# Matrixeigs/PowerSystemsReliabilityAssessment

Hardware: AMD Instinct MI355X
Metric: Monte Carlo DC-OPF scenarios/sec (RTS-24 HL2 non-sequential) (higher is better)
Workload: dtype f64

## Files before the change

powersystemsreliabilityassessment_amd/csrc/relmc_kernels.hip:

```cpp
#include "relmc_devfn.h"
#include "relmc_shape_rts24.h"

namespace relmc {


constexpr int kPrioBit = 12;
constexpr int kMinWaves = 2;
#define DINF __builtin_inf()
#define RELOAD_FENCE() __asm__ volatile("" ::: "memory")
#define SLOT_FENCE() __builtin_amdgcn_sched_barrier(0)
#ifdef RELMC_PASS_NOUNROLL
#define PASS_LOOP _Pragma("nounroll")
#else
#define PASS_LOOP
#endif
constexpr int kPfMask = 0xc0;
constexpr int kPfMaskWide = 0xc6;
#define PFSITE(k) (((PF_MASK >> (k)) & 1) != 0)
constexpr int kShadowMask = 0xff;
constexpr int kShadowMaskWide = 0xff;
constexpr int kNormSplitMask = 0xff;
constexpr int kNormSplitMaskWide = 0;
#ifdef RELMC_ZERO_EXPLICIT
constexpr bool kZeroBySlot = false;
#else
constexpr bool kZeroBySlot = true;
#endif
#ifdef RELMC_FILL_LOOP
constexpr bool kFillBySlot = false;
#else
constexpr bool kFillBySlot = true;
#endif
#define PASS_IDLE(d) (((d).x & 0xffffu) == ((d).y >> 16))
#define PASS_IDLE_INV(d) ((d).y != 0u)
#ifdef RELMC_PHASE_TIMING
#define PT_DECL unsigned long long pt_[8] = {0, 0, 0, 0, 0, 0, 0, 0}, ptn_[2] = {0, 0}; unsigned long long pt0_ = __builtin_readcyclecounter();
#define PT_MARK(k) { const unsigned long long n_ = __builtin_readcyclecounter(); pt_[k] += n_ - pt0_; pt0_ = n_; }
#define PT_TRIP(k) ptn_[k] += 1;
#define PT_FLUSH if (a.timing && lane == 0) { for (int k = 0; k < 8; ++k) a.timing[((size_t)blockIdx.x * WPB + (tid >> 6)) * 8 + k] = pt_[k]; \
                                              for (int k = 0; k < 2; ++k) a.timing[(size_t)gridDim.x * WPB * 8 + ((size_t)blockIdx.x * WPB + (tid >> 6)) * 2 + k] = ptn_[k]; }
#else
#define PT_DECL
#define PT_MARK(k)
#define PT_TRIP(k)
#define PT_FLUSH
#endif
#if defined(RELMC_PHASE_TIMING) && defined(RELMC_PT_INIT)
#undef PT_MARK
#define PT_MARK(k) { const unsigned long long n_ = __builtin_readcyclecounter(); pt_[(k) == 7 ? 7 : 6] += n_ - pt0_; pt0_ = n_; }
#define PT_IMARK(k) { const unsigned long long n_ = __builtin_readcyclecounter(); pt_[k] += n_ - pt0_; pt0_ = n_; }
#else
#define PT_IMARK(k)
#endif

template <int MODE_, class TL, class SH = ShapeDynamic>
__global__ void __launch_bounds__(64 * TL::WPB, kMinWaves) relmc_eval_kernel(const DevCaseT<TL>* __restrict__ gcase, const EvalArgs a)
{
    constexpr int MODE = MODE_ == 5 ? 0 : (MODE_ == 6 ? 4 : MODE_);
    constexpr bool DENSE = MODE_ == 6;
    constexpr int PAIR_MASK = TL::RW == 16 ? kRpairMask : kRpairMaskWide;
#define PAIRSITE(k) (((PAIR_MASK >> (k)) & 1) != 0)
    constexpr int PF_MASK = TL::RW == 16 ? kPfMask : kPfMaskWide;
    constexpr bool SHADOW = (((TL::RW == 16 ? kShadowMask : kShadowMaskWide) >> MODE) & 1) != 0;
    constexpr bool NSPLIT = (((TL::RW == 16 ? kNormSplitMask : kNormSplitMaskWide) >> MODE) & 1) != 0;
    constexpr bool LSHARE = (((TL::RW == 16 ? kLineRcpShareMask : kLineRcpShareMaskWide) >> MODE) & 1) != 0 && PAIRSITE(0) && PAIRSITE(2) && PAIRSITE(6);
    constexpr bool ZSLOT = kZeroBySlot && (SH::kMask & SH::grp_nl) != 0 && (SH::kMask & SH::grp_ninj) != 0;
    constexpr bool FSLOT = kFillBySlot && !DENSE && (SH::kMask & SH::grp_nzero_res) != 0 && (SH::kMask & SH::grp_nfill_bus) != 0;
    constexpr bool FBUS = FSLOT && SH::nfill_bus > 0;
    constexpr int RW = TL::RW, BS = TL::BS, LS = TL::LS, IS = TL::IS, NBT = TL::NBT, WPB = TL::WPB, SPW = TL::SPW, OW = TL::OW;
    using DevCase = DevCaseT<TL>;
    using Partial = PartialT<TL>;
    extern __shared__ __attribute__((aligned(16))) unsigned char smem[];
    constexpr uint32_t OPT_BYTES = 128;
    double* const OPT = reinterpret_cast<double*>(smem);
#define A_(k, name) OPT[k]
    DevCase& C = *reinterpret_cast<DevCase*>(smem + OPT_BYTES);
    const DevCase& TASKSRC = *gcase;
    const DevCase& TABL = C;
    const DevCase& TABI = (RW == 64) ? *gcase : C;
    const DevCase& TABG = (RW == 64) ? *gcase : C;
    const int tid = threadIdx.x, lane = tid & 63, rlane = lane & (RW - 1), row = tid / RW;
    const uint32_t case_bytes = a.case_bytes;
    {
        const uint32_t* src = reinterpret_cast<const uint32_t*>(gcase);
        uint32_t* dst = reinterpret_cast<uint32_t*>(smem + OPT_BYTES);
        if (tid == 0) { OPT[0] = a.feastol; OPT[1] = a.gradtol; OPT[2] = a.comptol; OPT[3] = a.costtol; OPT[4] = a.xi; OPT[5] = a.sigma;
                        OPT[6] = a.z0; OPT[7] = a.alpha_min; OPT[8] = a.max_stepsize; OPT[9] = a.fail_threshold; }
        if constexpr (FSLOT) {
            constexpr uint32_t LB0 = offsetof(DevCase, l_blk) / 4, LBN = sizeof(DevCase::l_blk) / 4, LF0 = offsetof(DevCase, l_blk_fill) / 4;
            static_assert(offsetof(DevCase, l_blk) % 4 == 0 && sizeof(DevCase::l_blk) % 4 == 0 && offsetof(DevCase, l_blk_fill) % 4 == 0, "l_blk and l_blk_fill are copied as 32-bit words");
            for (uint32_t i = tid; i < case_bytes / 4; i += 64 * WPB) dst[i] = src[i - LB0 < LBN ? LF0 + (i - LB0) : i];
        } else
        for (uint32_t i = tid; i < case_bytes / 4; i += 64 * WPB) dst[i] = src[i];
    }
    __syncthreads();
    double* const W = reinterpret_cast<double*>(smem + OPT_BYTES + ((case_bytes + 15u) & ~15u)) + (size_t)row * SHAPE(scen_doubles, a.scen_doubles);
    const int nlp = SHAPE(nl, C.nl), nip = SHAPE(ninj, C.ninj);
    double* const LR = W;
    double* const IR = W + 4 * (nlp + 1);
    const int maxdeg0 = SHAPE(maxdeg0, C.maxdeg_s[0]), maxdeg1 = SHAPE(maxdeg1, C.maxdeg_s[1]), maxinj0 = SHAPE(maxinj0, C.maxinj_s[0]), maxinj1 = SHAPE(maxinj1, C.maxinj_s[1]);
    double* const Stash = W + SHAPE(stash_off, a.stash_off) + 2 * rlane;
    const double* const StashJ = W + SHAPE(stash_off, a.stash_off);
    double* const Lam = W + SHAPE(stash_off, a.stash_off) + 2 * IS * RW + 2;
    uint32_t* const OB = reinterpret_cast<uint32_t*>(Lam + NBT);

    const int ng = SHAPE(ng, C.ng), ncomp = C.ncomp, nb = SHAPE(nb, C.nb);
    const bool bwd_all_half = SHAPE(bwd_all_half, __builtin_amdgcn_readfirstlane((uint32_t)(C.bwd_half != 0 ? 1u : 0u)) != 0);
    const int off_rhs = SHAPE(off_rhs, C.off_rhs), npu = SHAPE(npass_upd, C.npass_upd), npi = SHAPE(npass_inv, C.npass_inv), npass = SHAPE(npass, C.npass), nzero = SHAPE(nzero, C.nzero), npuh = SHAPE(npass_upd, C.npass_upd) - SHAPE(npass_updq, C.npass_updq), npuf = npuh - SHAPE(npass_updh, C.npass_updh);
    const double base = C.base_mva;
    const double eps = 2.220446049250313e-16;

    uint32_t linfo[LS]; int lpart[LS];
#pragma unroll
    for (int s = 0; s < LS; ++s) { const int l = RW * s + rlane; linfo[s] = C.l_info[l]; lpart[s] = C.l_partner[l]; }
    constexpr bool LTAB_LDS = (MODE == 1 || MODE == 2 || MODE == 4);
    constexpr bool ITAB_REG = RW == 64;
    double lbv_[LS], lrv_[LS], ihi_[IS], ilo_[IS];
#pragma unroll
    for (int s = 0; s < LS; ++s) { lbv_[s] = LTAB_LDS ? 0.0 : TABL.l_b[RW * s + rlane]; lrv_[s] = LTAB_LDS ? 0.0 : TABL.l_rate[RW * s + rlane]; }
#pragma unroll
    for (int s = 0; s < IS; ++s) { ihi_[s] = ITAB_REG ? TABI.i_tab[RW * s + rlane][0] : 0.0; ilo_[s] = ITAB_REG ? TABI.i_tab[RW * s + rlane][1] : 0.0; }
#define lb(s) (LTAB_LDS ? TABL.l_b[RW * (s) + rlane] : lbv_[s])
#define lr(s) (LTAB_LDS ? TABL.l_rate[RW * (s) + rlane] : lrv_[s])
#define IHL(s, j) (ITAB_REG ? d2{ihi_[s], ilo_[s]} : ld2(TABI.i_tab[j]))
#define ICOST(s, j) TABI.i_tab[j][2]
#define PLIST(t, bi) TABG.b_line8[bi]
#define JLIST(t, bi) TABG.b_inj8[bi]
    uint32_t iinfo[IS];
#pragma unroll
    for (int s = 0; s < IS; ++s) iinfo[s] = C.i_info[RW * s + rlane];
    int vb[BS];
#pragma unroll
    for (int t = 0; t < BS; ++t) vb[t] = FBUS ? (int)gcase->b_lane_fill[RW * t + rlane] : (int)C.b_lane[RW * t + rlane];

    Partial& PA = reinterpret_cast<Partial*>(a.partial)[(size_t)blockIdx.x * (64 * WPB) + tid];
    {
        PA.dns = 0.0; PA.dns2 = 0.0;
#pragma unroll
        for (int s = 0; s < IS; ++s) { PA.shed[s] = 0.0; PA.cf_inj[s] = 0; }
#pragma unroll
        for (int s = 0; s < LS; ++s) PA.cf_line[s] = 0;
        PA.n = 0; PA.nfail = 0; PA.nsing = 0; PA.ninf = 0; PA.nnc = 0; PA.iters = 0; PA.pad = 0;
    }
    uint32_t acc_n = 0, acc_it = 0;

    PT_DECL
    const int64_t ngroups = (a.n + SPW - 1) / SPW;
    const int64_t gwave = (int64_t)blockIdx.x * WPB + (tid >> 6);
    const int64_t gstride = (int64_t)gridDim.x * WPB;
    const bool prio_first = a.prio_mode == 1 ? blockIdx.x < (gridDim.x >> 1) : (a.prio_mode == 2 ? ((tid >> 8) & 1) == 0 : false);
    if (a.prio_mode != 0 && !prio_first) __builtin_amdgcn_s_setprio(1);
    constexpr bool WINDOWED = (MODE == 0 && RW == 16);
    uint32_t* const WIN = reinterpret_cast<uint32_t*>(smem + OPT_BYTES + ((case_bytes + 15u) & ~15u)) +
                          (size_t)SPW * WPB * SHAPE(scen_doubles, a.scen_doubles) * 2 + (size_t)(tid >> 6) * 256;
    uint8_t* const WINL = reinterpret_cast<uint8_t*>(smem + OPT_BYTES + ((case_bytes + 15u) & ~15u)) +
                          ((size_t)SPW * WPB * SHAPE(scen_doubles, a.scen_doubles) * 2 + (size_t)WPB * 256) * 4 + (size_t)(tid >> 6) * 64;
    int64_t wb_begin = gwave, wb_end = ngroups, wb_step = gstride;
    if (WINDOWED) {
        wb_begin = ngroups * gwave / gstride; wb_end = ngroups * (gwave + 1) / gstride; wb_step = 16;
    }
    static_assert(!WINDOWED || 80 + 4 * WPB <= OPT_BYTES, "one word per wavefront behind the ten option doubles");
    int* const TP = reinterpret_cast<int*>(smem + 80) + (tid >> 6);
    if (WINDOWED) { *TP = -1; RELOAD_FENCE(); }
    for (int64_t wb = wb_begin; WINDOWED || wb < wb_end; wb += wb_step) {
    int win_groups = 1, wg0 = 0;
    uint32_t win_valid = 0;
    if (WINDOWED) {
        const int T = a.tail_groups;
        int run = 16;
        if (__builtin_amdgcn_readfirstlane((int)(*TP < 0 && wb < wb_end - T)) != 0) {
            if (wb_end - T - wb < 16) run = (int)(wb_end - T - wb);
        } else {
            if (T == 0) break;
            uint32_t p = 0;
            if (lane == 0) p = atomicAdd(a.tail_count, 1u);
            p = __builtin_amdgcn_readfirstlane(p);
            int64_t n_ = a.n; uint32_t nw = gridDim.x;
            __asm__ volatile("" : "+s"(n_), "+s"(nw));
            nw *= WPB;
            if (p >= nw * (uint32_t)T) break;
            const int64_t ng_ = (n_ + SPW - 1) / SPW, owner = p % nw, ob = ng_ * owner / nw;
            wb_end = ng_ * (owner + 1) / nw;
            const int64_t g = wb_end - T + p / nw;
            wb = ob + ((g - ob) & ~(int64_t)15);
            wg0 = (int)(g - wb); run = wg0 + 1;
            *TP = (int)p;
            RELOAD_FENCE();
        }
        const int64_t si = wb * 4 + lane;
        const bool valid = (wb + (lane >> 2)) < wb_end && si < a.n;
        uint32_t m0 = 0, m1 = 0, m2 = 0, m3 = 0;
        bool hard = false;
        if (valid) {
            const uint64_t gi = a.first_index + (uint64_t)si;
            const int nblk = (ncomp + 3) >> 2;
            for (int blk = 0; blk < nblk; ++blk) {
                uint32_t w[4], nib = 0;
                philox4x32_10((uint32_t)gi, (uint32_t)(gi >> 32), (uint32_t)blk, 0u, (uint32_t)a.seed, (uint32_t)(a.seed >> 32), w);
#pragma unroll
                for (int e = 0; e < 4; ++e) {
                    const int k = blk * 4 + e;
                    if (k < ncomp && w[e] < C.thr[k]) nib |= 1u << e;
                }
                const uint32_t sh = nib << ((blk & 7) * 4);
                const int wsel = blk >> 3;
                if (wsel == 0) m0 |= sh; else if (wsel == 1) m1 |= sh; else if (wsel == 2) m2 |= sh; else m3 |= sh;
            }
            double cap = 0.0;
            for (int k = 0; k < ng; ++k) {
                const uint32_t wsel = k < 64 ? (k < 32 ? m0 : m1) : (k < 96 ? m2 : m3);
                if (!((wsel >> (k & 31)) & 1u)) cap += C.i_tab[k][0];
            }
            hard = cap * base < C.total_load;
        }
        const uint64_t bv = __ballot(valid), bh = __ballot(valid && hard);
        const uint64_t below = (1ull << lane) - 1ull;
        const uint32_t n_valid = (uint32_t)__popcll(bv), n_easy = (uint32_t)__popcll(bv & ~bh);
        if (valid) {
            const uint32_t slot = hard ? n_easy + (uint32_t)__popcll(bh & below) : (uint32_t)__popcll(bv & ~bh & below);
            uint4 pk; pk.x = m0; pk.y = m1; pk.z = m2; pk.w = m3;
            *reinterpret_cast<uint4*>(WIN + 4 * slot) = pk;
// ... 269 lines not shown
#pragma unroll
                            for (int s = 0; s < LS; ++s) {
                                if (L_ON(s)) {
                                    const int f = linfo[s] & 0xff, t = (linfo[s] >> 8) & 0xff;
                                    const int lf = LB[f], lt = LB[t];
                                    if (lf != lt) { ch = true; if (lf < lt) atomicMax(&LB[f], lt); else atomicMax(&LB[t], lf); }
                                }
                            }
                            RELOAD_FENCE();
                            if (!row_any<RW>(ch, lane)) break;
                        }
                    }
                    int ilab[IS];
#pragma unroll
                    for (int s = 0; s < IS; ++s) ilab[s] = any_lout ? LB[iinfo[s] & 0xff] : top;
#pragma unroll
                    for (int t = 0; t < BS; ++t) {
                        const int i = vb[t];
                        uint64_t roots = __ballot(i < nb && (any_lout ? LB[i] == i : i == top));
                        while (roots) {
                            const int pin = C.b_lane[RW * t + (int)__builtin_ctzll(roots)];
                            roots &= roots - 1;
                            bool inI[IS];
#pragma unroll
                            for (int s = 0; s < IS; ++s) inI[s] = I_ON(s) && ilab[s] == pin;
                            const bool dep = island_rules(inI);
#pragma unroll
                            for (int u = 0; u < BS; ++u)
                                if (vb[u] == pin) { sf |= 1u << (14 + u); if (dep) sf |= 1u << (16 + u); }
                            bf_top = dep ? 3 : 1;
                        }
                    }
#pragma unroll
                    for (int t = 0; t < BS; ++t) if (vb[t] < nb && any_lout) BF[vb[t]] = (B_PIN(t) ? 1 : 0) | (B_DROP(t) ? 2 : 0);
                    RELOAD_FENCE();
#pragma unroll
                    for (int s = 0; s < LS; ++s) {
                        if ((linfo[s] >> 24) & LF_EXISTS) {
                            const int f = linfo[s] & 0xff, t = (linfo[s] >> 8) & 0xff;
                            const int lo_b = f < t ? f : t, hi_b = f < t ? t : f;
                            const int flo = any_lout ? BF[lo_b] : (lo_b == top ? bf_top : 0), fhi = any_lout ? BF[hi_b] : (hi_b == top ? bf_top : 0);
                            if ((flo | fhi) & 1) sf |= 1u << (18 + s);
                            if ((fhi & 1) | (flo & 2)) sf |= 1u << (21 + s);
                            if ((flo & 1) | (fhi & 2)) sf |= 1u << (24 + s);
                        }
                    }
                    RELOAD_FENCE();
                }
            }

            PT_IMARK(3)
            uint32_t ow_p[LS];
            double t_lbp[LS];
#pragma unroll
            for (int s = 0; s < LS; ++s) {
                const int pr = (((linfo[s] >> 24) & LF_OWNER) && lpart[s] >= 0) ? lpart[s] : 0;
                ow_p[s] = OB[(ng + pr) >> 5]; t_lbp[s] = C.l_b[pr];
            }
            const double z0v = A_(6, z0);
#pragma unroll
            for (int s = 0; s < LS; ++s) {
                const uint32_t inf = linfo[s];
                if ((inf >> 24) & LF_OWNER) {
                    double v = L_ON(s) ? lb(s) : 0.0;
                    const int pr = lpart[s];
                    if (pr >= 0 && !((ow_p[s] >> ((ng + pr) & 31)) & 1u)) v += t_lbp[s];
                    cBv[s] = -v;
                }
            }
#pragma unroll
            for (int t = 0; t < BS; ++t) {
                const int i = vb[t];
                if (i < nb) {
                    double d = C.b_bsum[i];
                    if (any_lout) {
                        d = 0.0;
                        const int nlb = C.b_nline[i];
                        for (int e = 0; e < nlb; ++e) {
                            const int l = C.b_line[i][e] & 0x7f;
                            if (!outbit(OB, ng + l)) d += C.l_b[l];
                        }
                    }
                    cBd[t] = (B_PIN(t) || B_DROP(t)) ? 0.0 : d;
                }
            }

            PT_IMARK(4)
            const bool z0_small = __builtin_amdgcn_readfirstlane((int)(z0v < 1.0)) != 0;
            double fl = 0.0;
            uint32_t nq = 0;
#pragma unroll
            for (int s = 0; s < LS; ++s) {
                if (L_ACT(s)) {
                    const double h = -lr(s);
                    double z = z0v; if (h < -z0v) z = -h;
                    double mu = z0v; if (z0_small) { if (1.0 / z > z0v) mu = 1.0 / z; }
                    lzp[s] = z; lzm[s] = z; lmup[s] = mu; lmum[s] = mu;
                    nq += 2;
                }
            }
#pragma unroll
            for (int s = 0; s < IS; ++s) {
                if (I_ON(s)) {
                    const double hi = t_hi[s], lo = ILOV(s, t_lo[s]);
                    const bool box = hi - lo > eps;
                    if (box) sf |= 1u << (10 + s);
                    ip[s] = box ? 0.5 * (lo + hi) : hi;
                    if (box) {
                        const double h = -0.5 * (hi - lo);
                        double z = z0v; if (h < -z0v) z = -h;
                        double mu = z0v; if (z0_small) { if (1.0 / z > z0v) mu = 1.0 / z; }
                        izp[s] = z; izm[s] = z; imup[s] = mu; imum[s] = mu;
                        nq += 2;
                    }
                    fl += C.i_tab[RW * s + rlane][2] * ip[s];
                }
            }
#pragma unroll
            for (int t = 0; t < BS; ++t) if (vb[t] < nb) Lam[vb[t]] = 0.0;
            if (rlane == 0) st2(W + SHAPE(stash_off, a.stash_off) + 2 * IS * RW, 0.0, 0.0);
            niq = row_add<RW>(nq);
            fval = row_sum<RW>(fl);
            f0 = fval;
            iterating = !singular;
            status = singular ? 3 : 0;
        }

        PT_IMARK(5)
        PT_MARK(0)
        while (__any(iterating)) {
            if (prio_first) {
                if ((__builtin_readcyclecounter() >> kPrioBit) & 1ull) __builtin_amdgcn_s_setprio(3); else __builtin_amdgcn_s_setprio(0);
            }
            RELOAD_FENCE();
            if constexpr (RW == 16) {
                __asm__ volatile("" : "+v"(sf));
#pragma unroll
                for (int s = 0; s < LS; ++s) __asm__ volatile("" : "+v"(linfo[s]));
#pragma unroll
                for (int s = 0; s < IS; ++s) __asm__ volatile("" : "+v"(iinfo[s]));
#pragma unroll
                for (int t = 0; t < BS; ++t) __asm__ volatile("" : "+v"(vb[t]));
            }
#ifdef RELMC_TRACE
            const bool need_norms = true;
#else
            const bool need_norms = !NSPLIT || __builtin_amdgcn_readfirstlane((int)(__any(iterating && stage1) != 0 || a.norms_always != 0)) != 0;
#endif
            PT_TRIP(need_norms ? 1 : 0)
            auto front_half = [&](auto norms_c) __attribute__((always_inline)) {
                constexpr bool NORMS = decltype(norms_c)::value;
                double mx_gh = -DINF, mx_x = 0.0, mx_z = 0.0, mx_lx = 0.0, mx_lammu = 0.0;
                bool nanx = false;
                double gown[LS];
#pragma unroll
                for (int s = 0; s < LS; ++s) {
                    const int l = RW * s + rlane;
                    double g = 0.0, q = 0.0;
                    double lx = LGv[s];
                    if (L_ACT(s)) {
                        const double b = lb(s), rr = lr(s);
                        const double hp = LFv[s] - rr, hm = -LFv[s] - rr;
                        double rzp, rzm;
                        if constexpr (LSHARE) { lzr[s] = frcp(lzp[s] * lzm[s]); rzp = lzm[s] * lzr[s]; rzm = lzp[s] * lzr[s]; }
                        else frcp_pair<PAIRSITE(0)>(lzp[s], lzm[s], rzp, rzm);
                        g = b * b * (lmup[s] * rzp + lmum[s] * rzm);
                        lx = __builtin_fma(b, lmup[s] - lmum[s], lx);
                        q = b * ((lmup[s] * hp + gamma) * rzp - (lmum[s] * hm + gamma) * rzm);
                        if constexpr (NORMS) {
                            mx_gh = vmax(mx_gh, vmax(hp, hm));
                            mx_z = vmax(mx_z, vmax(lzp[s], lzm[s]));
                            mx_lammu = vmax(mx_lammu, vmax(lmup[s], lmum[s]));
                        }
                    }
                    gown[s] = g;
                    if (ZSLOT ? l <= nlp : l < nlp) { st2(LR + 4 * l, g, lx); st2(LR + 4 * l + 2, lx + q, LFv[s]); }
                    SLOT_FENCE();
                }
#pragma unroll
                for (int s = 0; s < IS; ++s) {
                    const int j = RW * s + rlane;
                    double invD = 0.0, npd = 0.0;
                    const double pv = ip[s];
                    if constexpr (!NSPLIT) { mx_x = vmax(mx_x, __builtin_fabs(pv)); nanx = nanx || pv != pv; }
                    if (I_BOX(s)) {
                        const d2 hl = IHL(s, j);
                        const double hp = pv - hl.x, hm = ILOV(s, hl.y) - pv;
                        const double lxp = ICOST(s, j) - Lam[iinfo[s] & 0xff] + (imup[s] - imum[s]);
                        if constexpr ((RW == 16 && kInjNform) || (RW == 64 && kInjNformWide)) {
                            const double N = __builtin_fma(imup[s], izm[s], imum[s] * izp[s]);
                            const double rN = frcp(N), zz = izp[s] * izm[s];
                            invD = zz * rN;
                            npd = __builtin_fma(lxp, zz, (imup[s] * hp + gamma) * izm[s] - (imum[s] * hm + gamma) * izp[s]) * rN;
                        } else {
                        double rzp, rzm; frcp_pair<PAIRSITE(1)>(izp[s], izm[s], rzp, rzm);
                        const double D = imup[s] * rzp + imum[s] * rzm;
                        const double np = lxp + (imup[s] * hp + gamma) * rzp - (imum[s] * hm + gamma) * rzm;
                        invD = frcp(D); npd = np * invD;
                        }
                        if constexpr (NORMS) {
                            mx_lx = vmax(mx_lx, __builtin_fabs(lxp));
                            mx_gh = vmax(mx_gh, vmax(hp, hm));
                            mx_z = vmax(mx_z, vmax(izp[s], izm[s]));
                            mx_lammu = vmax(mx_lammu, vmax(imup[s], imum[s]));
                        }
                    }
                    if (ZSLOT ? j <= nip : j < nip) IR[j] = pv;
                    st2(Stash + 2 * RW * s, invD, npd);
                    SLOT_FENCE();
                }
                PT_MARK(1)
                if (rlane == 0) {
                    if (!ZSLOT || nlp >= LS * RW) { st2(LR + 4 * nlp, 0.0, 0.0); st2(LR + 4 * nlp + 2, 0.0, 0.0); }
                    if (!ZSLOT || nip >= IS * RW) IR[nip] = 0.0;
                }
                uint32_t lblk_pf[LS]; uint32_t zo_pf = 0;
                if constexpr (PFSITE(1)) {
#pragma unroll
                    for (int s = 0; s < LS; ++s) lblk_pf[s] = C.l_blk[RW * s + rlane];
                    if constexpr (!FSLOT) zo_pf = C.zero_off[rlane];
                }
                unsigned long long pl_pf[BS], pj_pf[BS];
                if constexpr (PFSITE(2)) {
#pragma unroll
                    for (int t = 0; t < BS; ++t) { const int bq = vb[t] < nb ? vb[t] : 0; pl_pf[t] = PLIST(t, bq); pj_pf[t] = JLIST(t, bq); }
                }
                double vown[LS];
                {
                    double gp[LS];
#pragma unroll
                    for (int s = 0; s < LS; ++s) gp[s] = LR[4 * (lpart[s] >= 0 ? lpart[s] : nlp)];
#pragma unroll
                    for (int s = 0; s < LS; ++s) vown[s] = (((linfo[s] >> 24) & LF_OWNER) && !L_PIN(s)) ? -(gown[s] + gp[s]) : 0.0;
                }
                double d00[BS], d11[BS], r0[BS], r1[BS];
#pragma unroll
                for (int t = 0; t < BS; ++t) {
                    const int bi = vb[t];
                    d00[t] = 0; d11[t] = 0; r0[t] = 0; r1[t] = 0;
                    if (bi < nb) {
                        double md = 0.0, lx = 0.0, nq_ = 0.0, bal = 0.0, E = 0.0, ssum = 0.0;
                        const unsigned long long pl = PFSITE(2) ? pl_pf[t] : PLIST(t, bi), pj = PFSITE(2) ? pj_pf[t] : JLIST(t, bi);
#pragma unroll
                        for (int e = 0; e < DEGMAX; e += 2) {
                            if (e >= (t == 0 ? maxdeg0 : maxdeg1)) break;
                            const uint32_t ent0 = (uint32_t)(pl >> (8 * e)) & 0xffu, ent1 = (uint32_t)(pl >> (8 * e + 8)) & 0xffu;
                            const int l0 = (int)(ent0 & 0x7f), l1 = (int)(ent1 & 0x7f);
                            const double sg0 = (ent0 & 0x80) ? -1.0 : 1.0, sg1 = (ent1 & 0x80) ? -1.0 : 1.0;
                            const d2 ra0 = ld2(LR + 4 * l0), rb0 = ld2(LR + 4 * l0 + 2), ra1 = ld2(LR + 4 * l1), rb1 = ld2(LR + 4 * l1 + 2);
                            md += ra0.x;
                            lx = __builtin_fma(sg0, ra0.y, lx);
                            nq_ = __builtin_fma(sg0, rb0.x, nq_);
                            bal = __builtin_fma(sg0, rb0.y, bal);
                            md += ra1.x;
                            lx = __builtin_fma(sg1, ra1.y, lx);
                            nq_ = __builtin_fma(sg1, rb1.x, nq_);
                            bal = __builtin_fma(sg1, rb1.y, bal);
                        }
#pragma unroll
                        for (int e = 0; e < BINJMAX; e += 2) {
                            if (e >= (t == 0 ? maxinj0 : maxinj1)) break;
                            const int j0 = (int)((uint32_t)(pj >> (8 * e)) & 0xffu), j1 = (int)((uint32_t)(pj >> (8 * e + 8)) & 0xffu);
                            const d2 sh0 = ld2(StashJ + 2 * j0), sh1 = ld2(StashJ + 2 * j1);
                            const double p0 = IR[j0], p1 = IR[j1];
                            bal -= p0; E += sh0.x; ssum += sh0.y;
                            bal -= p1; E += sh1.x; ssum += sh1.y;
                        }
                        if (B_PIN(t)) {
                            d00[t] = 1.0; r0[t] = 0.0;
                            if constexpr (NORMS) mx_lammu = vmax(mx_lammu, __builtin_fabs(lx));
                        } else {
                            d00[t] = md; r0[t] = -nq_;
                            if constexpr (NORMS) mx_lx = vmax(mx_lx, __builtin_fabs(lx));
                        }
                        if (B_DROP(t)) {
                            d11[t] = -1.0; r1[t] = 0.0;
                        } else {
                            d11[t] = -E; r1[t] = -bal - ssum;
                            if constexpr (NORMS) {
                                mx_gh = vmax(mx_gh, __builtin_fabs(bal));
                                mx_lammu = vmax(mx_lammu, __builtin_fabs(bla[t]));
                            }
                        }
                        if constexpr (!NSPLIT) { mx_x = vmax(mx_x, __builtin_fabs(bth[t])); nanx = nanx || bth[t] != bth[t]; }
                    }
                }
                double o_ct = 0.0, o_cc = 0.0, o_am = 0.0;
                if constexpr (NSPLIT && PFSITE(7)) o_am = A_(7, alpha_min);
                RELOAD_FENCE();
                if constexpr (DENSE) {
                    const int n = 2 * nb, n1 = n + 1;
                    volatile double* A = a.dense + ((size_t)blockIdx.x * (WPB * SPW) + (size_t)(tid / RW)) * (size_t)a.dense_stride;
                    for (int e = rlane; e < n * n1; e += RW) A[e] = 0.0;
                    __threadfence_block();
#pragma unroll
                    for (int s = 0; s < LS; ++s) {
                        if ((linfo[s] >> 24) & LF_OWNER) {
                            const int f = linfo[s] & 0xff, t = (linfo[s] >> 8) & 0xff;
                            const int hi = f < t ? t : f, lo = f < t ? f : t;
                            const double c1 = L_C1Z(s) ? 0.0 : cBv[s], c2 = L_C2Z(s) ? 0.0 : cBv[s];
                            A[(2 * hi) * n1 + 2 * lo] = vown[s]; A[(2 * lo) * n1 + 2 * hi] = vown[s];
                            A[(2 * hi) * n1 + 2 * lo + 1] = c1; A[(2 * lo + 1) * n1 + 2 * hi] = c1;
                            A[(2 * hi + 1) * n1 + 2 * lo] = c2; A[(2 * lo) * n1 + 2 * hi + 1] = c2;
                        }
                    }
#pragma unroll
                    for (int t = 0; t < BS; ++t) {
                        const int bi = vb[t];
                        if (bi < nb) {
                            A[(2 * bi) * n1 + 2 * bi] = d00[t]; A[(2 * bi) * n1 + 2 * bi + 1] = cBd[t];
                            A[(2 * bi + 1) * n1 + 2 * bi] = cBd[t]; A[(2 * bi + 1) * n1 + 2 * bi + 1] = d11[t];
                            A[(2 * bi) * n1 + n] = r0[t]; A[(2 * bi + 1) * n1 + n] = r1[t];
                        }
                    }
                    __threadfence_block();
                } else {
#pragma unroll
                for (int s = 0; s < LS; ++s) {
                    const uint32_t lbf = FSLOT ? (PFSITE(1) ? lblk_pf[s] : (uint32_t)C.l_blk[RW * s + rlane]) : 0u;
                    if (FSLOT ? (SHAPE(nidle_line, 1) == 0 || lbf != 0xffffu) : ((linfo[s] >> 24) & LF_OWNER) != 0) {
                        const double c1 = L_C1Z(s) ? 0.0 : cBv[s];
                        const double c2 = L_C2Z(s) ? 0.0 : cBv[s];
                        double* blk = W + (FSLOT ? lbf : (PFSITE(1) ? lblk_pf[s] : (uint32_t)C.l_blk[RW * s + rlane]));
                        st2(blk, vown[s], c1); st2(blk + 2, c2, 0.0);
                    }
                }
                const int nzloop = FSLOT ? SHAPE(nzero_res, 0) : nzero;
                if constexpr (PFSITE(1) && !FSLOT) {
                    for (int z = rlane; z < nzero; z += RW) {
                        const uint32_t zn = C.zero_off[z + RW < TL::MAXOFF ? z + RW : z];
                        double* blk = W + zo_pf; st2(blk, 0.0, 0.0); st2(blk + 2, 0.0, 0.0);
                        zo_pf = zn;
                    }
                } else
                for (int z = rlane; z < nzloop; z += RW) { double* blk = W + C.zero_off[z]; st2(blk, 0.0, 0.0); st2(blk + 2, 0.0, 0.0); }
#pragma unroll
                for (int t = 0; t < BS; ++t) {
                    const int bi = vb[t];
                    if constexpr (FBUS) {
                        if ((t == 0 ? SHAPE(nidle_bus0, 1) : SHAPE(nidle_bus1, 1)) == 0 || bi != 0xffff) {
                            st2(W + 4 * bi, d00[t], cBd[t]); st2(W + 4 * bi + 2, cBd[t], d11[t]);
                            if (bi < nb) st2(W + off_rhs + 2 * bi, r0[t], r1[t]);
                        }
                    } else
                    if (bi < nb) {
                        st2(W + 4 * bi, d00[t], cBd[t]); st2(W + 4 * bi + 2, cBd[t], d11[t]);
                        st2(W + off_rhs + 2 * bi, r0[t], r1[t]);
                    }
                }
                }

                PT_MARK(2)
                bool conv = false, xnan = false;
                if constexpr (NSPLIT) {
                    mx_x = x_inf; xnan = x_nan;
                    conv = NORMS && stage1;
                } else {
                    if constexpr (PFSITE(7)) { o_ct = A_(2, comptol); o_cc = A_(3, costtol); o_am = A_(7, alpha_min); }
                    mx_x = row_max<RW>(mx_x);
                    xnan = row_any<RW>(nanx, lane);
                    if constexpr (!PFSITE(7)) { o_ct = A_(2, comptol); o_cc = A_(3, costtol); }
                    conv = it > 0 && zmu < o_ct * (1.0 + mx_x) && __builtin_fabs(fval - f0) < o_cc * (1.0 + __builtin_fabs(f0));
                }
#ifdef RELMC_TRACE
                {
                    const double t_gh = row_max<RW>(mx_gh), t_z = row_max<RW>(mx_z), t_lx = row_max<RW>(mx_lx), t_lm = row_max<RW>(mx_lammu);
                    if (a.timing && blockIdx.x == 0 && tid == 0 && it < 60) {
                        double* o = reinterpret_cast<double*>(a.timing) + 8 * it;
                        o[0] = t_gh / (1.0 + vmax(mx_x, t_z)); o[1] = t_lx / (1.0 + t_lm); o[2] = zmu / (1.0 + mx_x);
                        o[3] = __builtin_fabs(fval - f0) / (1.0 + __builtin_fabs(f0)); o[4] = alphap; o[5] = alphad; o[6] = gamma; o[7] = fval;
                    }
                }
#endif
                if constexpr (NORMS) if (__any(conv)) {
                    mx_gh = row_max<RW>(mx_gh); mx_z = row_max<RW>(mx_z); mx_lx = row_max<RW>(mx_lx); mx_lammu = row_max<RW>(mx_lammu);
                    conv = conv && mx_gh < A_(0, feastol) * (1.0 + vmax(mx_x, mx_z)) && mx_lx < A_(1, gradtol) * (1.0 + mx_lammu);
                }
                if (conv) { status = 0; iterating = false; }
                else if (it > 0 && (xnan || alphap < (PFSITE(7) ? o_am : A_(7, alpha_min)) || alphad < (PFSITE(7) ? o_am : A_(7, alpha_min)) || gamma < eps || gamma > 1.0 / eps)) { status = 2; iterating = false; }
                else if (it >= a.max_it) { status = 1; iterating = false; }
            };
            if (iterating) {
                if (need_norms) front_half(std::true_type{}); else front_half(std::false_type{});
            }
            PT_MARK(3)
            RELOAD_FENCE();
            if (iterating) {
                f0 = fval;
                it += 1;
                if constexpr (DENSE) {
                    const int n = 2 * nb, n1 = n + 1;
                    volatile double* A = a.dense + ((size_t)blockIdx.x * (WPB * SPW) + (size_t)(tid / RW)) * (size_t)a.dense_stride;
                    double* const Fm = W;
                    bool singular_k = false;
                    for (int k = 0; k < n; ++k) {
                        double best = -1.0; int bi = n;
                        for (int i = k + rlane; i < n; i += RW) { const double v = __builtin_fabs(A[(size_t)i * n1 + k]); if (v > best) { best = v; bi = i; } }
                        const double mx = row_max<RW>(best);
                        const uint32_t cand = (best == mx) ? (uint32_t)bi : (uint32_t)n;
                        const int p = (int)row_min_u32<RW>(cand);
                        if (!(mx > 0.0)) { singular_k = true; break; }
                        if (p != k) for (int j = k + rlane; j <= n; j += RW) { const double u = A[(size_t)k * n1 + j], v = A[(size_t)p * n1 + j]; A[(size_t)k * n1 + j] = v; A[(size_t)p * n1 + j] = u; }
                        __threadfence_block();
                        const double rp = 1.0 / A[(size_t)k * n1 + k];
                        for (int i = k + 1 + rlane; i < n; i += RW) Fm[i] = A[(size_t)i * n1 + k] * rp;
                        RELOAD_FENCE();
                        for (int i = k + 1; i < n; ++i) {
                            const double f = Fm[i];
                            if (f != 0.0) for (int j = k + 1 + rlane; j <= n; j += RW) A[(size_t)i * n1 + j] = A[(size_t)i * n1 + j] - f * A[(size_t)k * n1 + j];
                        }
                        __threadfence_block();
                    }
                    for (int k = n - 1; k >= 0 && !singular_k; --k) {
                        double sdot = 0.0;
                        for (int j = k + 1 + rlane; j < n; j += RW) sdot = __builtin_fma(A[(size_t)k * n1 + j], Fm[j], sdot);
                        sdot = row_sum<RW>(sdot);
                        if (rlane == 0) Fm[k] = (A[(size_t)k * n1 + n] - sdot) / A[(size_t)k * n1 + k];
                        RELOAD_FENCE();
                    }
                    double xs[(2 * NBT + RW - 1) / RW];
#pragma unroll
                    for (int q = 0; q < (2 * NBT + RW - 1) / RW; ++q) { const int e = rlane + RW * q; xs[q] = e < n ? (singular_k ? __builtin_nan("") : Fm[e]) : 0.0; }
                    RELOAD_FENCE();
#pragma unroll
                    for (int q = 0; q < (2 * NBT + RW - 1) / RW; ++q) { const int e = rlane + RW * q; if (e < n) W[off_rhs + e] = xs[q]; }
                    RELOAD_FENCE();
                } else {
                unsigned char* const W8 = reinterpret_cast<unsigned char*>(W);
#define WP(off) reinterpret_cast<double*>(W8 + (off))
#define SHADOW_PIN(...) do { if constexpr (SHADOW) __asm__ volatile("" :: __VA_ARGS__ : "memory"); } while (0)
                uint2 dsc = *reinterpret_cast<const uint2*>(&TASKSRC.task[0][rlane][0]);
                PASS_LOOP
                for (int p = 0; p < npuf; ++p) {
                    const uint2 nxt = *reinterpret_cast<const uint2*>(&TASKSRC.task[p + 1][rlane][0]);
                    const bool idle = PASS_IDLE(dsc);
                    if (SHADOW || !idle) {
                        const bool vec = (dsc.x & 0x8000u) != 0;
                        double* T = WP(dsc.x & 0x7fffu);
                        const double* Wa = WP(dsc.x >> 16);
                        const double* Wb = WP(dsc.y & 0xffffu);
                        const double* D = WP(dsc.y >> 16);
                        const d2 dA = ld2(D); const double dBy = D[3];
                        const d2 a0 = ld2(Wa), b0 = ld2(Wb), b1 = ld2(Wb + 2);
                        d2 t0 = ld2(T);
                        const double pm = dA.x, pb = dA.y, pe = -dBy;
                        const double q = frcp(__builtin_fma(pm, pe, pb * pb));
                        const double P00 = pe * q, P01 = pb * q, P11 = -pm * q;
                        const double g00 = __builtin_fma(a0.x, P00, a0.y * P01), g01 = __builtin_fma(a0.x, P01, a0.y * P11);
                        t0.x -= __builtin_fma(g00, b0.x, g01 * b0.y); t0.y -= __builtin_fma(g00, b1.x, g01 * b1.y);
                        SHADOW_PIN("v"(t0.x), "v"(t0.y)); if (!idle) st2(T, t0.x, t0.y);
                        if (SHADOW || !vec) {
                            const d2 a1 = ld2(Wa + 2);
                            d2 t1 = ld2(T + 2);
                            const double g10 = __builtin_fma(a1.x, P00, a1.y * P01), g11 = __builtin_fma(a1.x, P01, a1.y * P11);
                            t1.x -= __builtin_fma(g10, b0.x, g11 * b0.y); t1.y -= __builtin_fma(g10, b1.x, g11 * b1.y);
                            SHADOW_PIN("v"(t1.x), "v"(t1.y)); if (!idle && !vec) st2(T + 2, t1.x, t1.y);
                        }
                    }
                    dsc = nxt;
                }
                PASS_LOOP
                for (int p = npuf; p < npuh; ++p) {
                    const uint2 nxt = *reinterpret_cast<const uint2*>(&TASKSRC.task[p + 1][rlane][0]);
                    const bool idle = PASS_IDLE(dsc);
                    if (SHADOW || !idle) {
                        double* T = WP(dsc.x & 0xffffu);
                        const double* Wa = WP(dsc.x >> 16);
                        const double* Wb = WP(dsc.y & 0xffffu);
                        const double* D = WP(dsc.y >> 16);
                        const d2 dA = ld2(D); const double dBy = D[3];
                        const d2 a0 = ld2(Wa), b0 = ld2(Wb), b1 = ld2(Wb + 2);
                        d2 t0 = ld2(T);
                        const double pm = dA.x, pb = dA.y, pe = -dBy;
                        const double q = frcp(__builtin_fma(pm, pe, pb * pb));
                        const double P00 = pe * q, P01 = pb * q, P11 = -pm * q;
                        const double g00 = __builtin_fma(a0.x, P00, a0.y * P01), g01 = __builtin_fma(a0.x, P01, a0.y * P11);
                        t0.x -= __builtin_fma(g00, b0.x, g01 * b0.y); t0.y -= __builtin_fma(g00, b1.x, g01 * b1.y);
                        SHADOW_PIN("v"(t0.x), "v"(t0.y)); if (!idle) st2(T, t0.x, t0.y);
                    }
                    dsc = nxt;
                }
                PASS_LOOP
                for (int p = npuh; p < npu; ++p) {
                    const uint2 nxt = *reinterpret_cast<const uint2*>(&TASKSRC.task[p + 1][rlane][0]);
                    const bool idle = PASS_IDLE(dsc);
                    if (SHADOW || !idle) {
                        double* T = WP(dsc.x & 0xffffu);
                        const double* Wa = WP(dsc.x >> 16);
                        const double* Wb = WP(dsc.y & 0xffffu);
                        const double* D = WP(dsc.y >> 16);
                        const d2 dA = ld2(D); const double dBy = D[3];
                        const d2 a0 = ld2(Wa), b0 = ld2(Wb);
                        double t = *T;
                        const double pm = dA.x, pb = dA.y, pe = -dBy;
                        const double q = frcp(__builtin_fma(pm, pe, pb * pb));
                        const double P00 = pe * q, P01 = pb * q, P11 = -pm * q;
                        const double g0 = __builtin_fma(a0.x, P00, a0.y * P01), g1 = __builtin_fma(a0.x, P01, a0.y * P11);
                        t -= __builtin_fma(g0, b0.x, g1 * b0.y);
                        SHADOW_PIN("v"(t)); if (!idle) *T = t;
                    }
                    dsc = nxt;
                }
                PT_MARK(4)
                PASS_LOOP
                for (int p = npu; p < npu + npi; ++p) {
                    const uint2 nxt = *reinterpret_cast<const uint2*>(&TASKSRC.task[p + 1][rlane][0]);
                    const bool idle = PASS_IDLE_INV(dsc);
                    if (SHADOW || !idle) {
                        double* D = WP(dsc.x & 0xffffu);
                        double* Y = WP(dsc.x >> 16);
                        const d2 dA = ld2(D), y = ld2(Y); const double dBy = D[3];
                        const double pm = dA.x, pb = dA.y, pe = -dBy;
                        const double q = frcp(__builtin_fma(pm, pe, pb * pb));
                        const double P00 = pe * q, P01 = pb * q, P11 = -pm * q;
                        const double y0 = __builtin_fma(P00, y.x, P01 * y.y), y1 = __builtin_fma(P01, y.x, P11 * y.y);
                        SHADOW_PIN("v"(P00), "v"(P01), "v"(P11), "v"(y0), "v"(y1)); if (!idle) { st2(D, P00, P01); st2(D + 2, P01, P11); st2(Y, y0, y1); }
                    }
                    dsc = nxt;
                }
                PT_MARK(5)
                if (RW == 64 && bwd_all_half) {
                PASS_LOOP
                    for (int p = npu + npi; p < npass; ++p) {
                        const uint2 nxt = *reinterpret_cast<const uint2*>(&TASKSRC.task[p + 1][rlane][0]);
                        const bool idle = PASS_IDLE(dsc);
                        if (SHADOW || !idle) {
                            double* Yi = WP(dsc.x & 0xffffu);
                            const double* Wk = WP(dsc.x >> 16);
                            const double* Pr = WP(dsc.y & 0xffffu);
                            const double* Ya = WP(dsc.y >> 16);
                            const d2 w0 = ld2(Wk), w1 = ld2(Wk + 2), pr = ld2(Pr), x = ld2(Ya);
                            double y = *Yi;
                            const double u0 = __builtin_fma(w0.x, x.x, w1.x * x.y), u1 = __builtin_fma(w0.y, x.x, w1.y * x.y);
// ... 403 lines not shown
```

Measured before the change: 65.64 million.

## Test convergence before building the Newton system on norm iterations

Adds a two-stage form of the interior-point front half, used when norms are needed. It first computes only the residuals and norms needed for the convergence test. The expensive reciprocal, diagonal and RHS assembly then runs only if some lane is still iterating after the test. This skips the system build on the converging iteration, at the cost of an extra pass over the line and bus tables and a different shared-memory layout for the LR slots.

```diff
diff --git a/powersystemsreliabilityassessment_amd/csrc/relmc_kernels.hip b/powersystemsreliabilityassessment_amd/csrc/relmc_kernels.hip
--- a/powersystemsreliabilityassessment_amd/csrc/relmc_kernels.hip
+++ b/powersystemsreliabilityassessment_amd/csrc/relmc_kernels.hip
@@ -31,6 +31,11 @@
 #else
 constexpr bool kFillBySlot = true;
 #endif
+#ifdef RELMC_TEST_AFTER
+constexpr int kTestFirstMask = 0;
+#else
+constexpr int kTestFirstMask = 0x01;
+#endif
 #define PASS_IDLE(d) (((d).x & 0xffffu) == ((d).y >> 16))
 #define PASS_IDLE_INV(d) ((d).y != 0u)
 #ifdef RELMC_PHASE_TIMING
@@ -67,6 +72,8 @@
     constexpr bool ZSLOT = kZeroBySlot && (SH::kMask & SH::grp_nl) != 0 && (SH::kMask & SH::grp_ninj) != 0;
     constexpr bool FSLOT = kFillBySlot && !DENSE && (SH::kMask & SH::grp_nzero_res) != 0 && (SH::kMask & SH::grp_nfill_bus) != 0;
     constexpr bool FBUS = FSLOT && SH::nfill_bus > 0;
+    constexpr bool TFIRST = TL::RW == 16 && ((kTestFirstMask >> MODE) & 1) != 0 && NSPLIT && !DENSE && (SH::kMask & SH::grp_nl) != 0 && (SH::kMask & SH::grp_ninj) != 0 &&
+                            (SH::kMask & SH::grp_nzero_res) != 0 && (SH::kMask & SH::grp_nfill_bus) != 0;
     constexpr int RW = TL::RW, BS = TL::BS, LS = TL::LS, IS = TL::IS, NBT = TL::NBT, WPB = TL::WPB, SPW = TL::SPW, OW = TL::OW;
     using DevCase = DevCaseT<TL>;
     using Partial = PartialT<TL>;
@@ -642,7 +649,10 @@
                 constexpr bool NORMS = decltype(norms_c)::value;
                 double mx_gh = -DINF, mx_x = 0.0, mx_z = 0.0, mx_lx = 0.0, mx_lammu = 0.0;
                 bool nanx = false;
+                constexpr bool TF = TFIRST && NORMS;
+                static_assert(!TFIRST || (!PFSITE(1) && !PFSITE(2)), "the two-stage form reads its tables where it uses them");
                 double gown[LS];
+                if constexpr (!TF) {
 #pragma unroll
                 for (int s = 0; s < LS; ++s) {
                     const int l = RW * s + rlane;
@@ -667,6 +677,8 @@
                     if (ZSLOT ? l <= nlp : l < nlp) { st2(LR + 4 * l, g, lx); st2(LR + 4 * l + 2, lx + q, LFv[s]); }
                     SLOT_FENCE();
                 }
+                }
+                if constexpr (!TF) {
 #pragma unroll
                 for (int s = 0; s < IS; ++s) {
                     const int j = RW * s + rlane;
@@ -699,11 +711,12 @@
                     st2(Stash + 2 * RW * s, invD, npd);
                     SLOT_FENCE();
                 }
+                }
                 PT_MARK(1)
-                if (rlane == 0) {
+                if constexpr (!TF) { if (rlane == 0) {
                     if (!ZSLOT || nlp >= LS * RW) { st2(LR + 4 * nlp, 0.0, 0.0); st2(LR + 4 * nlp + 2, 0.0, 0.0); }
                     if (!ZSLOT || nip >= IS * RW) IR[nip] = 0.0;
-                }
+                } }
                 uint32_t lblk_pf[LS]; uint32_t zo_pf = 0;
                 if constexpr (PFSITE(1)) {
 #pragma unroll
@@ -716,7 +729,7 @@
                     for (int t = 0; t < BS; ++t) { const int bq = vb[t] < nb ? vb[t] : 0; pl_pf[t] = PLIST(t, bq); pj_pf[t] = JLIST(t, bq); }
                 }
                 double vown[LS];
-                {
+                if constexpr (!TF) {
                     double gp[LS];
 #pragma unroll
                     for (int s = 0; s < LS; ++s) gp[s] = LR[4 * (lpart[s] >= 0 ? lpart[s] : nlp)];
@@ -724,6 +737,7 @@
                     for (int s = 0; s < LS; ++s) vown[s] = (((linfo[s] >> 24) & LF_OWNER) && !L_PIN(s)) ? -(gown[s] + gp[s]) : 0.0;
                 }
                 double d00[BS], d11[BS], r0[BS], r1[BS];
+                if constexpr (!TF) {
 #pragma unroll
                 for (int t = 0; t < BS; ++t) {
                     const int bi = vb[t];
@@ -775,6 +789,80 @@
                         if constexpr (!NSPLIT) { mx_x = vmax(mx_x, __builtin_fabs(bth[t])); nanx = nanx || bth[t] != bth[t]; }
                     }
                 }
+                }
+                if constexpr (TFIRST) { if constexpr (TF) {
+#pragma unroll
+                    for (int s = 0; s < LS; ++s) {
+                        const int l = RW * s + rlane;
+                        double lx = LGv[s];
+                        if (L_ACT(s)) {
+                            const double b = lb(s), rr = lr(s);
+                            const double hp = LFv[s] - rr, hm = -LFv[s] - rr;
+                            lx = __builtin_fma(b, lmup[s] - lmum[s], lx);
+                            mx_gh = vmax(mx_gh, vmax(hp, hm));
+                            mx_z = vmax(mx_z, vmax(lzp[s], lzm[s]));
+                            mx_lammu = vmax(mx_lammu, vmax(lmup[s], lmum[s]));
+                        }
+                        if (ZSLOT ? l <= nlp : l < nlp) st2(LR + 4 * l, lx, LFv[s]);
+                        SLOT_FENCE();
+                    }
+#pragma unroll
+                    for (int s = 0; s < IS; ++s) {
+                        const int j = RW * s + rlane;
+                        const double pv = ip[s];
+                        if (I_BOX(s)) {
+                            const d2 hl = IHL(s, j);
+                            const double hp = pv - hl.x, hm = ILOV(s, hl.y) - pv;
+                            const double lxp = ICOST(s, j) - Lam[iinfo[s] & 0xff] + (imup[s] - imum[s]);
+                            mx_lx = vmax(mx_lx, __builtin_fabs(lxp));
+                            mx_gh = vmax(mx_gh, vmax(hp, hm));
+                            mx_z = vmax(mx_z, vmax(izp[s], izm[s]));
+                            mx_lammu = vmax(mx_lammu, vmax(imup[s], imum[s]));
+                        }
+                        if (ZSLOT ? j <= nip : j < nip) IR[j] = pv;
+                        SLOT_FENCE();
+                    }
+                    PT_MARK(1)
+                    if (rlane == 0) {
+                        if (!ZSLOT || nlp >= LS * RW) { st2(LR + 4 * nlp, 0.0, 0.0); st2(LR + 4 * nlp + 2, 0.0, 0.0); }
+                        if (!ZSLOT || nip >= IS * RW) IR[nip] = 0.0;
+                    }
+#pragma unroll
+                    for (int t = 0; t < BS; ++t) {
+                        const int bi = vb[t];
+                        r1[t] = 0.0;
+                        if (bi < nb) {
+                            double lx = 0.0, bal = 0.0;
+                            const unsigned long long pl = PLIST(t, bi), pj = JLIST(t, bi);
+#pragma unroll
+                            for (int e = 0; e < DEGMAX; e += 2) {
+                                if (e >= (t == 0 ? maxdeg0 : maxdeg1)) break;
+                                const uint32_t ent0 = (uint32_t)(pl >> (8 * e)) & 0xffu, ent1 = (uint32_t)(pl >> (8 * e + 8)) & 0xffu;
+                                const int l0 = (int)(ent0 & 0x7f), l1 = (int)(ent1 & 0x7f);
+                                const double sg0 = (ent0 & 0x80) ? -1.0 : 1.0, sg1 = (ent1 & 0x80) ? -1.0 : 1.0;
+                                const d2 ra0 = ld2(LR + 4 * l0), ra1 = ld2(LR + 4 * l1);
+                                lx = __builtin_fma(sg0, ra0.x, lx);
+                                bal = __builtin_fma(sg0, ra0.y, bal);
+                                lx = __builtin_fma(sg1, ra1.x, lx);
+                                bal = __builtin_fma(sg1, ra1.y, bal);
+                            }
+#pragma unroll
+                            for (int e = 0; e < BINJMAX; e += 2) {
+                                if (e >= (t == 0 ? maxinj0 : maxinj1)) break;
+                                const int j0 = (int)((uint32_t)(pj >> (8 * e)) & 0xffu), j1 = (int)((uint32_t)(pj >> (8 * e + 8)) & 0xffu);
+                                const double p0 = IR[j0], p1 = IR[j1];
+                                bal -= p0;
+                                bal -= p1;
+                            }
+                            if (B_PIN(t)) mx_lammu = vmax(mx_lammu, __builtin_fabs(lx)); else mx_lx = vmax(mx_lx, __builtin_fabs(lx));
+                            if (!B_DROP(t)) {
+                                mx_gh = vmax(mx_gh, __builtin_fabs(bal));
+                                mx_lammu = vmax(mx_lammu, __builtin_fabs(bla[t]));
+                            }
+                            r1[t] = bal;
+                        }
+                    }
+                } }
                 double o_ct = 0.0, o_cc = 0.0, o_am = 0.0;
                 if constexpr (NSPLIT && PFSITE(7)) o_am = A_(7, alpha_min);
                 RELOAD_FENCE();
@@ -804,7 +892,7 @@
                         }
                     }
                     __threadfence_block();
-                } else {
+                } else if constexpr (!TF) {
 #pragma unroll
                 for (int s = 0; s < LS; ++s) {
                     const uint32_t lbf = FSLOT ? (PFSITE(1) ? lblk_pf[s] : (uint32_t)C.l_blk[RW * s + rlane]) : 0u;
@@ -869,6 +957,117 @@
                 if (conv) { status = 0; iterating = false; }
                 else if (it > 0 && (xnan || alphap < (PFSITE(7) ? o_am : A_(7, alpha_min)) || alphad < (PFSITE(7) ? o_am : A_(7, alpha_min)) || gamma < eps || gamma > 1.0 / eps)) { status = 2; iterating = false; }
                 else if (it >= a.max_it) { status = 1; iterating = false; }
+                if constexpr (TFIRST) { if constexpr (TF) { if (__any(iterating)) { if (iterating) {
+#pragma unroll
+                    for (int s = 0; s < LS; ++s) {
+                        const int l = RW * s + rlane;
+                        double g = 0.0, q = 0.0;
+                        double lx = LGv[s];
+                        if (L_ACT(s)) {
+                            const double b = lb(s), rr = lr(s);
+                            const double hp = LFv[s] - rr, hm = -LFv[s] - rr;
+                            double rzp, rzm;
+                            if constexpr (LSHARE) { lzr[s] = frcp(lzp[s] * lzm[s]); rzp = lzm[s] * lzr[s]; rzm = lzp[s] * lzr[s]; }
+                            else frcp_pair<PAIRSITE(0)>(lzp[s], lzm[s], rzp, rzm);
+                            g = b * b * (lmup[s] * rzp + lmum[s] * rzm);
+                            lx = __builtin_fma(b, lmup[s] - lmum[s], lx);
+                            q = b * ((lmup[s] * hp + gamma) * rzp - (lmum[s] * hm + gamma) * rzm);
+                        }
+                        gown[s] = g;
+                        if (ZSLOT ? l <= nlp : l < nlp) st2(LR + 4 * l + 2, g, lx + q);
+                        SLOT_FENCE();
+                    }
+#pragma unroll
+                    for (int s = 0; s < IS; ++s) {
+                        const int j = RW * s + rlane;
+                        double invD = 0.0, npd = 0.0;
+                        const double pv = ip[s];
+                        if (I_BOX(s)) {
+                            const d2 hl = IHL(s, j);
+                            const double hp = pv - hl.x, hm = ILOV(s, hl.y) - pv;
+                            const double lxp = ICOST(s, j) - Lam[iinfo[s] & 0xff] + (imup[s] - imum[s]);
+                            if constexpr ((RW == 16 && kInjNform) || (RW == 64 && kInjNformWide)) {
+                                const double N = __builtin_fma(imup[s], izm[s], imum[s] * izp[s]);
+                                const double rN = frcp(N), zz = izp[s] * izm[s];
+                                invD = zz * rN;
+                                npd = __builtin_fma(lxp, zz, (imup[s] * hp + gamma) * izm[s] - (imum[s] * hm + gamma) * izp[s]) * rN;
+                            } else {
+                                double rzp, rzm; frcp_pair<PAIRSITE(1)>(izp[s], izm[s], rzp, rzm);
+                                const double D = imup[s] * rzp + imum[s] * rzm;
+                                const double np = lxp + (imup[s] * hp + gamma) * rzp - (imum[s] * hm + gamma) * rzm;
+                                invD = frcp(D); npd = np * invD;
+                            }
+                        }
+                        st2(Stash + 2 * RW * s, invD, npd);
+                        SLOT_FENCE();
+                    }
+                    {
+                        double gp[LS];
+#pragma unroll
+                        for (int s = 0; s < LS; ++s) gp[s] = LR[4 * (lpart[s] >= 0 ? lpart[s] : nlp) + 2];
+#pragma unroll
+                        for (int s = 0; s < LS; ++s) vown[s] = (((linfo[s] >> 24) & LF_OWNER) && !L_PIN(s)) ? -(gown[s] + gp[s]) : 0.0;
+                    }
+#pragma unroll
+                    for (int t = 0; t < BS; ++t) {
+                        const int bi = vb[t];
+                        const double bal = r1[t];
+                        d00[t] = 0; d11[t] = 0; r0[t] = 0; r1[t] = 0;
+                        if (bi < nb) {
+                            double md = 0.0, nq_ = 0.0, E = 0.0, ssum = 0.0;
+                            const unsigned long long pl = PLIST(t, bi), pj = JLIST(t, bi);
+#pragma unroll
+                            for (int e = 0; e < DEGMAX; e += 2) {
+                                if (e >= (t == 0 ? maxdeg0 : maxdeg1)) break;
+                                const uint32_t ent0 = (uint32_t)(pl >> (8 * e)) & 0xffu, ent1 = (uint32_t)(pl >> (8 * e + 8)) & 0xffu;
+                                const int l0 = (int)(ent0 & 0x7f), l1 = (int)(ent1 & 0x7f);
+                                const double sg0 = (ent0 & 0x80) ? -1.0 : 1.0, sg1 = (ent1 & 0x80) ? -1.0 : 1.0;
+                                const d2 rb0 = ld2(LR + 4 * l0 + 2), rb1 = ld2(LR + 4 * l1 + 2);
+                                md += rb0.x;
+                                nq_ = __builtin_fma(sg0, rb0.y, nq_);
+                                md += rb1.x;
+                                nq_ = __builtin_fma(sg1, rb1.y, nq_);
+                            }
+#pragma unroll
+                            for (int e = 0; e < BINJMAX; e += 2) {
+                                if (e >= (t == 0 ? maxinj0 : maxinj1)) break;
+                                const int j0 = (int)((uint32_t)(pj >> (8 * e)) & 0xffu), j1 = (int)((uint32_t)(pj >> (8 * e + 8)) & 0xffu);
+                                const d2 sh0 = ld2(StashJ + 2 * j0), sh1 = ld2(StashJ + 2 * j1);
+                                E += sh0.x; ssum += sh0.y;
+                                E += sh1.x; ssum += sh1.y;
+                            }
+                            if (B_PIN(t)) { d00[t] = 1.0; r0[t] = 0.0; } else { d00[t] = md; r0[t] = -nq_; }
+                            if (B_DROP(t)) { d11[t] = -1.0; r1[t] = 0.0; } else { d11[t] = -E; r1[t] = -bal - ssum; }
+                        }
+                    }
+                    RELOAD_FENCE();
+#pragma unroll
+                    for (int s = 0; s < LS; ++s) {
+                        const uint32_t lbf = (uint32_t)C.l_blk[RW * s + rlane];
+                        if (FSLOT ? (SHAPE(nidle_line, 1) == 0 || lbf != 0xffffu) : ((linfo[s] >> 24) & LF_OWNER) != 0) {
+                            const double c1 = L_C1Z(s) ? 0.0 : cBv[s], c2 = L_C2Z(s) ? 0.0 : cBv[s];
+                            double* blk = W + lbf;
+                            st2(blk, vown[s], c1); st2(blk + 2, c2, 0.0);
+                        }
+                    }
+                    const int nzloop = FSLOT ? SHAPE(nzero_res, 0) : nzero;
+                    for (int z = rlane; z < nzloop; z += RW) { double* blk = W + C.zero_off[z]; st2(blk, 0.0, 0.0); st2(blk + 2, 0.0, 0.0); }
+#pragma unroll
+                    for (int t = 0; t < BS; ++t) {
+                        const int bi = vb[t];
+                        if constexpr (FBUS) {
+                            if ((t == 0 ? SHAPE(nidle_bus0, 1) : SHAPE(nidle_bus1, 1)) == 0 || bi != 0xffff) {
+                                st2(W + 4 * bi, d00[t], cBd[t]); st2(W + 4 * bi + 2, cBd[t], d11[t]);
+                                if (bi < nb) st2(W + off_rhs + 2 * bi, r0[t], r1[t]);
+                            }
+                        } else
+                        if (bi < nb) {
+                            st2(W + 4 * bi, d00[t], cBd[t]); st2(W + 4 * bi + 2, cBd[t], d11[t]);
+                            st2(W + off_rhs + 2 * bi, r0[t], r1[t]);
+                        }
+                    }
+                    PT_MARK(2)
+                } } } }
             };
             if (iterating) {
                 if (need_norms) front_half(std::true_type{}); else front_half(std::false_type{});
```

Result: faster. 66.52 million, median of 6 (+1.3%).
